# NomaDamas/AutoRAG-Research

Measured on AMD Instinct MI355X. Metric: queries/sec, higher is better.
Workload: dtype f32

## Files before the change

### autorag_research_amd/csrc/index.h

```cpp
#pragma once
#include <climits>
#include <hip/hip_runtime.h>

#include <algorithm>
#include <cmath>
#include <cstdio>
#include <cstring>
#include <mutex>
#include <string>
#include <vector>

#include "dev_common.h"
#include "mi355dr.h"

namespace mi355 {
template <class T, bool Pinned = false>
struct DevBuf {
    T* p = nullptr;
    size_t bytes = 0;
    DevBuf() = default;
    DevBuf(const DevBuf&) = delete;
    DevBuf& operator=(const DevBuf&) = delete;
    ~DevBuf() { release(); }
    void release() {
        if (p) (void)(Pinned ? hipHostFree(p) : hipFree(p));
        p = nullptr;
        bytes = 0;
    }
    hipError_t grow(size_t want) {
        if (want <= bytes) return hipSuccess;
        void* q = nullptr;
        const hipError_t e = Pinned ? hipHostMalloc(&q, want) : hipMalloc(&q, want);
        if (e != hipSuccess) return e;
        release();
        p = (T*)q;
        bytes = want;
        return hipSuccess;
    }
    void swap(DevBuf& o) {
        std::swap(p, o.p);
        std::swap(bytes, o.bytes);
    }
    operator T*() const { return p; }
};
template <class T>
using HostBuf = DevBuf<T, true>;

// ... 28 lines not shown
    int k = 0;
    int level = 0;
    bool screening = false;
    bool i8 = false;
    bool wide = false;
    int cap = 0;
    bool speculative = false;
    bool spec_eligible = false;
    int spec_m = 0;
    const char* refused = nullptr;
};
struct Pending {
    bool active = false;
    Event done;
    HostBuf<int> status_host;
    hipStream_t stream = nullptr;
    const float* q_dev = nullptr;
    int B = 0;
    Pass pass;
    double* out_dist = nullptr;
    int64_t* out_rows = nullptr;
};
struct RetryBufs {
    DevBuf<float> q;
    DevBuf<double> dist;
    DevBuf<int64_t> rows;
    DevBuf<int> map;
};
constexpr int kPendingRing = 4;

// ... 327 lines not shown
```

### autorag_research_amd/csrc/k_prep.h

```cpp
#pragma once
#include "dev_common.h"

namespace mi355 {

__global__ __launch_bounds__(64) void k_row_nrm2(const float* __restrict__ rows, int64_t row0, int64_t n, int d,
                                                  float* __restrict__ nrm2, unsigned* __restrict__ n2max,
                                                  const int64_t* __restrict__ ids) {
    __shared__ float tile[kStageFloats];
    const int lane = threadIdx.x;
    const int64_t j = (int64_t)blockIdx.x * kWave + lane;
    const bool live = j < n;
    const int64_t i = ids ? (live ? ids[j] : 0) : row0 + j;
    const float* my_row = live ? rows + i * (int64_t)d : nullptr;
    float acc = 0.0f;
    for (int k0 = 0; k0 < d; k0 += kStageCols) {
        stage_rows(tile, my_row, k0, d, lane);
        __syncthreads();
        const int kn = min(kStageCols, d - k0);
        const float* t = tile + lane * kStageLd;
        for (int k = 0; k < kn; ++k) acc = __builtin_fmaf(t[k], t[k], acc);
        __syncthreads();
    }
    if (live) nrm2[i] = acc;
    float m = (live && norm_is_regular(acc)) ? acc : 0.0f;
// ... 133 lines not shown
            if (!tight && i >= first_new) {
                const int slot = atomicAdd(irr8_count, 1);
                if (slot < kIrrCap) irr8_rows[slot] = (int32_t)i;
            }
        }
    }
    __syncthreads();
    if (threadIdx.x == 0) {
        float mx = 0.0f;
        for (int j = 0; j < kI8GroupRows; ++j) mx = fmaxf(mx, s_err[j]);
        grp[g].step = step;
        grp[g].err = mx;
    }
}

__global__ __launch_bounds__(64) void k_prep_queries(const float* __restrict__ q, int B, int d, int dpad, int metric,
                                                      QueryState st, int dpad8, int i8, float bf16_ec, int* status_or,
                                                      int* prune_skip, int cnt0, float cscale) {
    extern __shared__ float qs[];
    const int b = blockIdx.x;
    const int lane = threadIdx.x;
    if (b == 0 && lane == 0) {
        if (status_or) *status_or = 0;
        if (prune_skip) prune_skip[0] = prune_skip[1] = 0;
    }
    uint16_t* qh = st.qhat + (int64_t)b * dpad;
    if (b >= B) {
        for (int k = lane; k < dpad; k += kWave) qh[k] = 0;
        if (lane == 0) {
            st.qn[b] = 0.0f;
            st.thr[b] = __builtin_inff();
            st.cnt[b] = 0;
            st.carry[b] = 0;
            st.thr_used[b] = -__builtin_inff();
            st.best_n[b] = 0;
            st.thr_key[b] = 0;
            st.thr_row[b] = -1;
            st.status[b] = 0;
            st.E[b] = bf16_screen_bound(0.00390625f, bf16_ec, d, cscale);
            st.E16[b] = st.E[b];
            st.sc[b] = 0.0f;
            st.kq[b] = 1.0f;
        }
        if (i8)
            for (int k = lane; k < dpad8; k += kWave) st.qhat8[(int64_t)b * dpad8 + k] = 0;
        return;
    }
    const float* qr = q + (int64_t)b * d;
    for (int k = lane; k < d; k += kWave) qs[k] = qr[k];
    __syncthreads();
    float acc = 0.0f;
    for (int k = 0; k < d; ++k) acc = __builtin_fmaf(qs[k], qs[k], acc);
    const bool regular = norm_is_regular(acc);
    const float rq = regular ? 1.0f / sqrtf(acc) : 0.0f;
    float eq2 = 0.0f;
    for (int k = lane; k < dpad; k += kWave) {
        uint16_t v = 0;
        if (k < d && regular) {
            const float qh_f = qs[k] * rq;
            v = f32_to_bf16_rn(qh_f);
            const float e = qh_f - bf16_bits_to_f32(v);
            eq2 = __builtin_fmaf(e, e, eq2);
        }
        qh[k] = v;
// ... 50 lines not shown
```

### autorag_research_amd/csrc/k_select.h

```cpp
#pragma once
#include "dev_common.h"

namespace mi355 {

struct PruneArgs {
    const float* rows;
    const float* nrm2;
    const float* q;
    QueryState st;
    int32_t* cand_row;
    float* cand_val;
    const int* qlist;
    unsigned long long* stat;
    int cap, d, k, metric;
    int exact;
    const uint8_t* flag8;
    float cscale;
    const uint16_t* shadow16;
    int dpad;
    int round_a;
    int* skip_list;
    int skip_parity;
    int thr_only;
    int one_wave_only;
    int defer_b;
    SpecModel spec;
};

__device__ __forceinline__ float unit_sim(int metric, double dist, float inv_qn) {
    return metric == 0 ? (float)(1.0 - dist) : (float)(-dist) * inv_qn;
}
__device__ __forceinline__ float screen_threshold(int metric, double dist_k, float E, float nq) {
    if (metric == 0) return float_below((float)((1.0 - dist_k) - (double)E));
    const double u = -dist_k / sqrt((double)nq);
    return float_below((float)(u - fabs(u) * 4e-6 - (double)E));
}

constexpr int kPruneSmallThreads = 64, kPruneSmallSort = 1024;
constexpr int kPruneBigThreads = 256, kPruneBigSort = kSortMax;

__host__ __device__ inline size_t prune_qs_floats(int d) { return ((size_t)d + 3) / 4 * 4 + 16; }
// ... 37 lines not shown
        }
    }
#pragma unroll
    for (int j = 0; j < PER; ++j) {
        uint32_t kk = 0;
        if (j * T + tid < n_new) {
            if (v[j] != v[j]) kk = 0xFFFFFFFFu;
            else if (!f[j]) kk = f32_order_key(v[j]);
        }
        key[j] = kk;
        if (ROWS) rows_out[j] = r[j];
    }
}

template <int THREADS, int SORT>
__device__ __forceinline__ void prune_body(const PruneArgs& a, char* smem);

template <int THREADS, int SORT>
__global__ __launch_bounds__(THREADS) void k_prune(PruneArgs a) {
    extern __shared__ __attribute__((aligned(16))) char smem[];
    const bool list_mode = a.skip_list != nullptr && a.qlist == nullptr;
    const int tid = threadIdx.x;
    const int lane = tid & 63, wave = tid >> 6;
    int q = a.qlist ? a.qlist[blockIdx.x] : blockIdx.x;
    if (SORT == kPruneBigSort && list_mode) {
        if (blockIdx.x == 0 && tid == 0) a.skip_list[a.skip_parity ^ 1] = 0;
        const int n_left = a.skip_list[a.skip_parity];
        for (int i = blockIdx.x; i < n_left; i += gridDim.x) {
            PruneArgs b = a;
            b.skip_list = nullptr;
            b.qlist = a.skip_list + 2 + a.skip_parity * kQBlockMax + i - 0;
            b.qlist -= blockIdx.x;
            prune_body<THREADS, SORT>(b, smem);
            __syncthreads();
        }
        return;
    }
    prune_body<THREADS, SORT>(a, smem);
}

template <int THREADS, int SORT>
__device__ __forceinline__ void prune_body(const PruneArgs& a, char* smem) {
    constexpr int kWaves = THREADS / kWave;
    uint64_t* SK = (uint64_t*)smem;
    int32_t* SR = (int32_t*)(smem + (size_t)SORT * 8);
    char* X = smem + (size_t)SORT * 12;
    constexpr size_t xa = (size_t)kWaves * kStageFloats * sizeof(float), xb = (size_t)SORT * sizeof(float);
    constexpr size_t xbytes = xa > xb ? xa : xb;
    float* Lf = (float*)X;
    float* tiles = (float*)X;
    int32_t* R = (int32_t*)(X + xbytes);
    float* qs = (float*)(X + xbytes + (size_t)SORT * 4);
    int& s_cnt = *(int*)(X + xbytes + (size_t)SORT * 4 + (prune_qs_floats(a.d) - 16) * 4);
    float* q16 = qs + prune_qs_floats(a.d);
    const bool list_mode = a.skip_list != nullptr && a.qlist == nullptr;
    const int q = a.qlist ? a.qlist[blockIdx.x] : blockIdx.x;
    const int tid = threadIdx.x;
    const int lane = tid & 63, wave = tid >> 6;
    const int raw_cnt = a.st.cnt[q];
    const int n_best = a.st.best_n[q];
    if (raw_cnt == 0) return;
    if (a.exact && SORT < kPruneBigSort) return;
    auto leave_for_general = [&]() {
        if (a.one_wave_only) {
            if (tid == 0) {
                a.st.status[q] |= kStOverflow;
                a.st.cnt[q] = 0;
            }
            return;
        }
        if (list_mode && tid == 0) {
            const int i = atomicAdd(&a.skip_list[a.skip_parity], 1);
            a.skip_list[2 + a.skip_parity * kQBlockMax + i] = q;
        }
    };
    if (raw_cnt > a.cap) {
        if (SORT < kPruneBigSort) {
            leave_for_general();
            return;
        }
        if (tid == 0) {
            a.st.status[q] |= kStOverflow;
            a.st.cnt[q] = 0;
        }
        return;
    }
    if (n_best + raw_cnt > SORT) {
        if (SORT < kPruneBigSort) {
            leave_for_general();
            return;
        }
        if (tid == 0) {
            a.st.status[q] |= kStOverflow;
            a.st.cnt[q] = 0;
        }
        return;
    }
    const int n_new = raw_cnt;
    const int32_t* crow = a.cand_row + (int64_t)q * a.cap;
    const float* cval = a.cand_val + (int64_t)q * a.cap;
    uint64_t* bkey = a.st.best_key + (int64_t)q * kKMax;
    int32_t* brow = a.st.best_row + (int64_t)q * kKMax;
    const float nq = a.st.qn[q];
    const float inv_qn = 1.0f / sqrtf(nq);
    const float E = a.st.E[q];
    if (tid == 0) {
        a.stat[2 * q] += (unsigned long long)(n_new - a.st.carry[q]);
        a.st.carry[q] = 0;
    }

    int n_res;
// ... 204 lines not shown
                        a.st.thr_key[q] = wk;
                        a.st.thr_row[q] = R2[a.k - 1];
                    }
                    if (wk != kKeyNaN && !(a.st.status[q] & kStIrregular)) {
                        float thr = screen_threshold(a.metric, key_to_dist(wk), E, nq);
                        if (a.thr_only && a.spec.moments != nullptr) {
                            const double dist_t = a.metric == 0 ? 1.0 - (double)t_model : -(double)t_model * sqrt((double)nq);
                            const float thr_model = screen_threshold(a.metric, dist_t, E, nq);
                            if (thr_model > thr && thr_model < __builtin_inff()) thr = thr_model;
                            a.st.thr_used[q] = thr;
                        }
                        a.st.thr[q] = thr;
                    }
                }
            }
            return;
        }
    }
    if (!a.exact) {
        const int nLp = next_pow2(n_new);
        for (int i = tid; i < nLp; i += THREADS) {
            float v = -__builtin_inff();
            if (i < n_new) {
                v = cval[i];
                if (v != v) v = __builtin_inff();
                else if (a.flag8 && a.flag8[crow[i]]) v = -__builtin_inff();
            }
            Lf[i] = v;
            R[i] = i;
        }
        if (tid == 0) s_cnt = 0;
// ... 86 lines not shown
    for (int i = tid; i < n_keep; i += THREADS) {
        bkey[i] = SK[i];
        brow[i] = SR[i];
    }
    if (tid == 0) {
        a.st.best_n[q] = n_keep;
        a.st.cnt[q] = 0;
        if (n_keep >= a.k) {
            const uint64_t wk = SK[a.k - 1];
            a.st.thr_key[q] = wk;
            a.st.thr_row[q] = SR[a.k - 1];
            if (!a.exact && wk != kKeyNaN && !(a.st.status[q] & kStIrregular))
                a.st.thr[q] = screen_threshold(a.metric, key_to_dist(wk), E, nq);
        }
    }
}

__global__ __launch_bounds__(64) void k_emit_irregular(const int32_t* __restrict__ irr_rows, int irr_n, QueryState st,
                                                        int32_t* cand_row, float* cand_val, int cap, int skip_below) {
    const int q = blockIdx.x;
    if (st.status[q] & kStIrregular) return;
    for (int i = threadIdx.x; i < irr_n; i += blockDim.x) {
        if (irr_rows[i] < skip_below) continue;
        const int slot = atomicAdd(&st.cnt[q], 1);
        if (slot < cap) {
            cand_row[(int64_t)q * cap + slot] = irr_rows[i];
            cand_val[(int64_t)q * cap + slot] = __builtin_nanf("");
        }
    }
}

__global__ __launch_bounds__(64) void k_finalize(QueryState st, int k, int64_t row_offset, const int64_t* __restrict__ row_map,
                                                  double* out_dist, int64_t* out_rows, int* status_or, int spec_metric) {
    const int q = blockIdx.x;
    const int n = st.best_n[q];
    if (threadIdx.x == 0 && spec_metric >= 0 && !(st.status[q] & kStIrregular)) {
        float thr_final = -__builtin_inff();
        if (n >= k) {
            const uint64_t wk = st.best_key[(int64_t)q * kKMax + k - 1];
            if (wk != kKeyNaN) thr_final = screen_threshold(spec_metric, key_to_dist(wk), st.E[q], st.qn[q]);
        }
        if (n < k || thr_final < st.thr_used[q]) st.status[q] |= kStSpecMiss;
    }
    for (int s = threadIdx.x; s < k; s += blockDim.x) {
        if (s < n && st.best_row[(int64_t)q * kKMax + s] != kRowNone) {
            out_dist[(int64_t)q * k + s] = key_to_dist(st.best_key[(int64_t)q * kKMax + s]);
            const int32_t r = st.best_row[(int64_t)q * kKMax + s];
            out_rows[(int64_t)q * k + s] = row_map ? row_map[r] : (int64_t)r + row_offset;
        } else {
            out_dist[(int64_t)q * k + s] = __longlong_as_double(0x7FF8000000000000ll);
            out_rows[(int64_t)q * k + s] = -1;
        }
    }
    if (threadIdx.x == 0 && st.status[q] != 0) atomicOr(status_or, st.status[q]);
}

__global__ __launch_bounds__(256) void k_merge_topk(const double* __restrict__ dist_all,
                                                     const int64_t* __restrict__ rows_all, int64_t rank_stride, int world,
                                                     int B, int k, double* out_dist, int64_t* out_rows) {
    extern __shared__ __attribute__((aligned(16))) char smem[];
    uint64_t* SK = (uint64_t*)smem;
    const int np_ = next_pow2(world * k);
    int32_t* SI = (int32_t*)(smem + (size_t)np_ * 8);
    const int q = blockIdx.x;
    const int n = world * k;
    const int np = next_pow2(n);
    for (int i = threadIdx.x; i < np; i += blockDim.x) {
        if (i < n) {
            const int w = i / k, s = i % k;
            const int64_t src = (int64_t)w * rank_stride + (int64_t)q * k + s;
// ... 58 lines not shown
```

### autorag_research_amd/csrc/mi355dr.hip

```cpp
#include "index.h"
#include "k_prep.h"
#include "k_scan.h"
#include "k_scan_ids.h"
#include "subset_ids.h"
#include "screen_common.h"
#include "k_screen.h"
#include "k_screen256c.h"
#include "k_screen_rq.h"

#define MI355_RQ_FORMS(X) X(1) X(2) X(3) X(4) X(5) X(6)
inline bool screen_rq_has(int ksteps) { return ksteps >= 1 && ksteps <= 6; }
#include "k_screen_stream.h"
#include "k_select.h"
#include "k_prune_wide.h"
#include "k_update.h"
#include "k_compact.h"
#include "k_view.h"
#include "k_block.h"
#include "k_mmr.h"
#include "mmr_order.h"
#include "k_groups.h"
#include "k_fuse.h"
#include "k_range.h"
#include "k_rows.h"
// ... 225 lines not shown
    ps.screening = idx->n > 0 && screen_possible && path != MI355DR_PATH_SCAN;
    ps.wide = ps.screening && wide_ok(idx, k);
    ps.cap = !idx->cap_set && ps.wide ? kCandCapWide : idx->cap;
    if (idx->screen_dtype == MI355DR_SCREEN_I8 && !i8_available(idx) && path != MI355DR_PATH_SCAN)
        ps.refused = "int8 screen unavailable: too many rows outside the residual limit";
    else if (path == MI355DR_PATH_SCREEN && !screen_possible && idx->n > 0) ps.refused = no_screen;
    ps.spec_m = spec_m_of(k);
    ps.spec_eligible = level == 0 && ps.screening && !ps.wide && ps.spec_m > 0 && idx->speculate && idx->n >= idx->spec_min_rows &&
                       kSpecInflation * ps.spec_m * 4 <= 3 * (std::min(kPruneSmallSort, ps.cap) - k) &&
                       starter_sample_rows(idx, ps) > 0;
    ps.speculative = ps.spec_eligible && idx->spec_probation <= 0;
    return ps;
}
inline bool idle_i8(const mi355dr_index* idx) { return decide_pass(idx, idx->last_pass_k, 0, false).i8; }

int launch_prune(mi355dr_index* idx, hipStream_t s, const Pass& ps, int nblocks, const int* qlist, int exact,
                 bool thr_only = false, bool one_wave_only = false, bool defer_b = false, const SpecModel* spec = nullptr) {
    PruneArgs pa{};
    if (spec) pa.spec = *spec;
    pa.thr_only = thr_only ? 1 : 0;
    pa.one_wave_only = one_wave_only ? 1 : 0;
    pa.defer_b = defer_b && idx->defer_round_b ? 1 : 0;
    pa.rows = idx->rows;
    pa.nrm2 = idx->nrm2;
    pa.q = idx->qdev;
    pa.st = idx->st;
    pa.cand_row = idx->cand_row;
    pa.cand_val = idx->cand_val;
    pa.qlist = qlist;
    pa.stat = idx->stat_dev;
    pa.cap = ps.cap;
    pa.d = idx->dim;
    pa.k = ps.k;
    pa.metric = idx->metric;
    pa.exact = exact;
    pa.flag8 = (ps.i8 && (idx->irr8_n > 0 || idx->dead_n > 0)) ? idx->flag8 : nullptr;
    pa.cscale = idx->metric == MI355DR_METRIC_IP ? idx->cmax : 1.0f;
    pa.shadow16 = (ps.i8 && idx->metric == 0 && !exact && idx->prefilter16) ? idx->shadow : nullptr;
    pa.dpad = idx->dpad;
    pa.round_a = idx->round_a;
    if (!exact && ps.wide) {
        pa.shadow16 = nullptr;
        hipLaunchKernelGGL((k_prune_wide<2, 32>), dim3(nblocks), dim3(2 * kWave), prune_wide_lds_bytes(idx->dim, 2), s, pa);
        HIPCHECK(idx, hipGetLastError());
        return MI355DR_OK;
    }
    if (pa.cap > kCandCap) return fail(idx, MI355DR_E_INTERNAL, "general-form prune on a list stride above kCandCap");
    const bool list_mode = qlist == nullptr;
    pa.skip_list = list_mode ? idx->prune_skip : nullptr;
    pa.skip_parity = list_mode ? (idx->prune_parity ^= 1) : 0;
    hipLaunchKernelGGL((k_prune<kPruneSmallThreads, kPruneSmallSort>), dim3(nblocks), dim3(kPruneSmallThreads),
                       prune_lds_bytes(idx->dim, kPruneSmallThreads, kPruneSmallSort, pa.shadow16 ? idx->dpad : 0), s, pa);
    HIPCHECK(idx, hipGetLastError());
    if (one_wave_only) return MI355DR_OK;
    hipLaunchKernelGGL((k_prune<kPruneBigThreads, kPruneBigSort>), dim3(list_mode ? std::min(nblocks, 64) : nblocks),
                       dim3(kPruneBigThreads), prune_lds_bytes(idx->dim, kPruneBigThreads, kPruneBigSort, 0), s, pa);
    HIPCHECK(idx, hipGetLastError());
    return MI355DR_OK;
}

int launch_prep(mi355dr_index* idx, hipStream_t s, int B, int Bpad, int metric, bool i8, int cnt0 = 0) {
    hipLaunchKernelGGL(k_prep_queries, dim3(Bpad), dim3(64), (size_t)idx->dim * sizeof(float), s, idx->qdev, B, idx->dim,
                       idx->dpad, metric, idx->st, idx->dpad8, i8 ? 1 : 0, idx->bf16_ec, idx->status_or_dev,
                       idx->prune_skip, cnt0, idx->metric == MI355DR_METRIC_IP ? idx->cmax : 1.0f);
    idx->prune_parity = 0;
    HIPCHECK(idx, hipGetLastError());
    return MI355DR_OK;
}

inline int screen_tile(int B) { return B > kTileN ? kT2 : kTileM; }

constexpr int kRetryLevels = 2;

enum ScreenKernel { kKernTile = 0, kKernStream = 1, kKern256c = 2, kKernRq = 3 };
inline ScreenKernel screen_kernel_for(const mi355dr_index* idx, bool i8, int B, int64_t rows, bool emit_all) {
    const int tile = (emit_all || rows <= idx->small_chunk_rows) ? kTileM : screen_tile(B);
    const int row_bytes = i8 ? idx->dpad8 : idx->dpad * 2;
    const int ksteps = row_bytes / kRowB;
    if (tile == kT2) return i8 && idx->screen_rq && screen_rq_has(ksteps) ? kKernRq : kKern256c;
// ... 173 lines not shown
    const double zq = normal_quantile(1.0 - (double)ps.spec_m / (double)idx->n) + idx->spec_shift_milli / 1000.0;
    sm.zq = (float)zq;
    if (zq_out) *zq_out = zq;
    return sm;
}

PassPlan make_plan(const mi355dr_index* idx, const Pass& ps, int B) {
    const double budget = growth_budget(idx, ps.k, ps.i8);
    double growth = std::max(0.25, std::min((double)idx->chunk_growth, budget));
    if (B <= 64 && ps.level == 0 && idx->chunk_growth_set == 0) growth = std::max(growth, std::min(8.0, budget * kSmallBlockBudget));
    if (ps.level == 1) growth = std::max(0.25, growth * 0.5);
    if (ps.level >= 2) growth = 0.25;
    return plan_pass(idx, ps, B, growth);
}

int run_screen(mi355dr_index* idx, hipStream_t s, const Pass& ps, int B, const PassPlan& plan) {
    int64_t kept_all_below = 0;
    const bool i8 = ps.i8;
    const int side_n = i8 ? idx->irr8_n : idx->irr_n;
    constexpr int kSideMerge = 32;
    bool side_done = false;
    const bool lean = plan.sample > 0 && idx->prune_companion == 0;
    auto timed = [&](bool big, int64_t rows, auto&& launch) -> int {
        EventPair ev{};
        if (idx->profile) {
            ev = take_events(idx);
            HIPCHECK(idx, hipEventRecord(ev.a, s));
        }
        CHECK(launch());
        if (idx->profile) {
            HIPCHECK(idx, hipEventRecord(ev.b, s));
// ... 23 lines not shown
    }
    int64_t done = 0;
    for (size_t ci = 0; ci < plan.ends.size(); ++ci) {
        const int64_t end = plan.ends[ci];
        const bool emit_all = ci == 0 && plan.emit_all_first;
        if (emit_all) kept_all_below = end;
        const bool big = !emit_all && end - done > idx->small_chunk_rows && screen_tile(B) == kT2;
        const int64_t seen = ci == 0 ? (plan.sample > 0 ? plan.sample : end) : done;
        const double lanes = ps.speculative ? (double)kSpecInflation * ps.spec_m * 4096.0 / (double)idx->n
                                            : 8.0 * ps.k * 4096.0 / (double)std::max<int64_t>(seen, 1);
        int period = 1;
        while (period < 64 && period * 2 * lanes <= idx->screen_flush_lanes) period *= 2;
        const int flush_mask = idx->screen_flush_sync ? period - 1 : -1;
        CHECK(timed(big, end - done, [&] { return launch_screen(idx, s, i8, B, done, end, ps.cap, emit_all ? kEmitAll : 0, flush_mask); }));
        idx->s_chunks++;
        if (end >= idx->n && side_n > 0 && side_n <= kSideMerge) {
            hipLaunchKernelGGL(k_emit_irregular, dim3(B), dim3(64), 0, s, i8 ? idx->irr8_rows : idx->irr_rows, side_n, idx->st,
                               idx->cand_row, idx->cand_val, ps.cap, (int)kept_all_below);
            HIPCHECK(idx, hipGetLastError());
            side_done = true;
        }
        const bool last = end >= idx->n && (side_n == 0 || side_done);
        CHECK(launch_prune(idx, s, ps, B, nullptr, 0, false, lean, !last));
        done = end;
    }
    if (side_n > 0 && !side_done) {
        hipLaunchKernelGGL(k_emit_irregular, dim3(B), dim3(64), 0, s, i8 ? idx->irr8_rows : idx->irr_rows, side_n, idx->st,
                           idx->cand_row, idx->cand_val, ps.cap, (int)kept_all_below);
        HIPCHECK(idx, hipGetLastError());
        CHECK(launch_prune(idx, s, ps, B, nullptr, 0, false, lean));
    }
    idx->s_passes++;
    return MI355DR_OK;
}

int launch_scan(mi355dr_index* idx, hipStream_t s, const int* qlist, int nq, int cap, int64_t r0, int64_t r1,
                const int32_t* ids = nullptr) {
    ScanArgs sa{};
    sa.rows = idx->rows;
    sa.nrm2 = idx->nrm2;
    sa.q = idx->qdev;
    sa.st = idx->st;
    sa.cand_row = idx->cand_row;
    sa.cand_val = idx->cand_val;
    sa.qlist = qlist;
// ... 57 lines not shown
                }
            }
            done = end;
            chunk = std::max<int64_t>(chunk, done * (idx->chunk_growth_set ? idx->chunk_growth : 63));
        }
    }
    if (ids) HIPCHECK(idx, hipStreamSynchronize(s));
    else idx->s_fallback_queries += nq_all;
    return MI355DR_OK;
}

int subset_block(mi355dr_index* idx, hipStream_t s, const float* q_dev, int B, int k, int64_t m, double* out_dist_dev,
                 int64_t* out_rows_dev) {
    const Pass ps = decide_pass(idx, k, 0, true);
    idx->last_pass_k = k;
    if (q_dev != idx->qdev)
        HIPCHECK(idx, hipMemcpyAsync(idx->qdev, q_dev, (size_t)B * idx->dim * sizeof(float), hipMemcpyDeviceToDevice, s));
    CHECK(launch_prep(idx, s, B, (int)round_up(B, screen_tile(B)), idx->metric, ps.i8));
    std::vector<int> all(B);
    for (int i = 0; i < B; ++i) all[i] = i;
    if (m > 0) CHECK(run_scan(idx, s, ps, all, m, idx->subset_ids));
    hipLaunchKernelGGL(k_finalize, dim3(B), dim3(64), 0, s, idx->st, k, idx->row_offset, idx->view_row_map.p, out_dist_dev,
                       out_rows_dev, idx->status_or_dev, -1);
    HIPCHECK(idx, hipGetLastError());
    HIPCHECK(idx, hipMemcpyAsync(idx->status_host, idx->st.status, (size_t)kQBlockMax * sizeof(int), hipMemcpyDeviceToHost, s));
    HIPCHECK(idx, hipStreamSynchronize(s));
    for (int i = 0; i < B; ++i)
        if (idx->status_host[i] & kStOverflow)
            return fail(idx, MI355DR_E_INTERNAL, "subset scan: query " + std::to_string(i) + " lost a candidate chunk");
    return MI355DR_OK;
}

int pending_alloc(mi355dr_index* idx, Pending& p) {
    HIPCHECK(idx, p.status_host.grow((kQBlockMax + 1) * sizeof(int)));
    HIPCHECK(idx, p.done.create(hipEventDisableTiming));
    return MI355DR_OK;
}

int enqueue_block(mi355dr_index* idx, hipStream_t s, const float* q_dev, int B, int k, double* out_dist_dev,
                  int64_t* out_rows_dev, Pending& p, int level = 0, bool force_scan = false) {
    CHECK(ensure_qstate(idx));
    CHECK(pending_alloc(idx, p));
    idx->last_pass_k = k;
    if (level == 0 && idx->screen_dtype == MI355DR_SCREEN_AUTO && k >= idx->i8_demoted_k && --idx->i8_probation <= 0)
        idx->i8_demoted_k = INT_MAX;
    const int Bpad = (int)round_up(B, screen_tile(B));
    const Pass ps = decide_pass(idx, k, level, force_scan, "screen path unavailable (metric or too many irregular rows)");
    if (ps.refused) return fail(idx, MI355DR_E_UNSUPPORTED, ps.refused);
    if (idx->spec_probation > 0 && ps.spec_eligible) idx->spec_probation--;
    if (q_dev != idx->qdev)
        HIPCHECK(idx, hipMemcpyAsync(idx->qdev, q_dev, (size_t)B * idx->dim * sizeof(float), hipMemcpyDeviceToDevice, s));
    PassPlan plan;
    if (ps.screening) plan = make_plan(idx, ps, B);
    CHECK(launch_prep(idx, s, B, Bpad, idx->metric, ps.i8, starter_count(plan)));
    if (idx->n > 0) {
        if (ps.screening) {
            CHECK(run_screen(idx, s, ps, B, plan));
        } else {
            std::vector<int> all(B);
            for (int i = 0; i < B; ++i) all[i] = i;
            CHECK(run_scan(idx, s, ps, all, idx->n));
        }
    }
    hipLaunchKernelGGL(k_finalize, dim3(B), dim3(64), 0, s, idx->st, k, idx->row_offset, idx->view_row_map.p, out_dist_dev,
                       out_rows_dev, idx->status_or_dev, ps.speculative && idx->n > 0 ? idx->metric : -1);
    HIPCHECK(idx, hipGetLastError());
    HIPCHECK(idx, hipMemcpyAsync(p.status_host, idx->st.status, (size_t)(kQBlockMax + 1) * sizeof(int), hipMemcpyDeviceToHost, s));
    HIPCHECK(idx, hipEventRecord(p.done, s));
    p.active = true;
    p.stream = s;
    p.q_dev = q_dev;
    p.B = B;
    p.pass = ps;
    p.out_dist = out_dist_dev;
    p.out_rows = out_rows_dev;
    return MI355DR_OK;
}

int search_block(mi355dr_index* idx, hipStream_t s, const float* q_dev, int B, int k, double* out_dist_dev,
                 int64_t* out_rows_dev, int level = 0, bool force_scan = false);

int complete_block(mi355dr_index* idx, Pending& p) {
    if (!p.active) return MI355DR_OK;
    p.active = false;
    HIPCHECK(idx, hipEventSynchronize(p.done));
    drain_events(idx);
    if (!p.pass.screening) {
        for (int i = 0; i < p.B; ++i)
            if (p.status_host[i] & kStOverflow)
                return fail(idx, MI355DR_E_INTERNAL, "exact scan: query " + std::to_string(i) + " lost a candidate chunk");
        return MI355DR_OK;
    }
    if (p.status_host[kQBlockMax] == 0) return MI355DR_OK;
    hipStream_t s = p.stream;
    const int B = p.B, k = p.pass.k, level = p.pass.level;
    std::vector<int> sub;
    int n_todo = 0;
    {
        std::vector<int> retry;
        for (int i = 0; i < B; ++i) {
            const int st = p.status_host[i];
            if (st == 0) continue;
            if (p.pass.speculative && !(st & kStIrregular)) {
                if (st & kStOverflow) idx->s_spec_overflow_queries++;
                else if (st & kStSpecMiss) idx->s_spec_miss_queries++;
            }
            if (level < kRetryLevels && !(st & kStIrregular)) retry.push_back(i);
            else sub.push_back(i);
// ... 1245 lines not shown

int range_block(mi355dr_index* idx, hipStream_t s, const float* q_dev, int nb, const double* radius, int m, double* od,
                int64_t* orow, int64_t* ocount) {
    const Pass ps = decide_pass(idx, 1, 0, false, "screen path unavailable (too many irregular rows)");
    if (ps.refused) return fail(idx, MI355DR_E_UNSUPPORTED, ps.refused);
    const int cap = ps.cap;
    const bool i8 = ps.i8, use_screen = ps.screening;
    const int64_t chunk = round_up(std::max<int64_t>(idx->range_chunk_rows, kT2), kT2);
    std::vector<RangeSpan> spans;
    for (int64_t r0 = 0; r0 < idx->n; r0 += chunk) spans.push_back(RangeSpan{r0, std::min(idx->n, r0 + chunk)});
    const int n_main = (int)spans.size();
    const int R = range_slots_for(idx, m);
    const int64_t pairs = (int64_t)nb * std::max(n_main, 1);
    CHECK(ensure_range(idx, nb, R, m, pairs));
    const RangeState rs = range_state(idx, R, pairs);
    if (q_dev != idx->qdev)
        HIPCHECK(idx, hipMemcpyAsync(idx->qdev, q_dev, (size_t)nb * idx->dim * sizeof(float), hipMemcpyDeviceToDevice, s));
    CHECK(launch_prep(idx, s, nb, (int)round_up(nb, screen_tile(nb)), idx->metric, i8));
    HIPCHECK(idx, hipMemcpyAsync(idx->rng.radius.p, radius, (size_t)nb * sizeof(double), hipMemcpyHostToDevice, s));
    HIPCHECK(idx, hipMemsetAsync(idx->rng.redo.p, 0, 2 * sizeof(int), s));
    HIPCHECK(idx, hipMemsetAsync(idx->rng.stat.p, 0, 2 * sizeof(unsigned long long), s));
    hipLaunchKernelGGL(k_range_prep, dim3((nb + kRangeThreads - 1) / kRangeThreads), dim3(kRangeThreads), 0, s,
                       (const double*)idx->rng.radius.p, nb, idx->metric, use_screen ? 1 : 0, idx->st, rs);
    HIPCHECK(idx, hipGetLastError());
    std::vector<int> all(nb);
    for (int i = 0; i < nb; ++i) all[i] = i;
    if (use_screen) {
        for (int i = 0; i < n_main; ++i) {
            CHECK(launch_screen(idx, s, i8, nb, spans[i].r0, spans[i].r1, cap, 0, idx->screen_flush_sync ? 15 : -1));
            CHECK(launch_range_collect(idx, s, ps, rs, kRangeFormScreen, nb, nullptr, i, spans[i].r0));
        }
        const int side_n = i8 ? idx->irr8_n : idx->irr_n;
        const int32_t* side = i8 ? idx->irr8_rows.p : idx->irr_rows.p;
// ... 141 lines not shown
    for (int b0 = 0; b0 < B; b0 += kQBlockMax) {
        const int nb = std::min(kQBlockMax, B - b0);
        const BlockOut<int64_t> o = block_outputs(idx, io, b0);
        HIPCHECK(idx, hipMemcpyAsync(idx->rowq.ids.p, row_ids + b0, (size_t)nb * sizeof(int64_t), hipMemcpyHostToDevice, s));
        hipLaunchKernelGGL(k_rows_gather, dim3(nb), dim3(kRowsThreads), 0, s, (const int64_t*)idx->rowq.ids.p, idx->row_offset,
                           idx->n, (const float*)idx->rows.p, (const float*)idx->nrm2.p, idx->dim, idx->rowq.q.p,
                           idx->rowq.valid.p, idx->rowq.pair_q.p, idx->rowq.pair_row.p, idx->rowq.skipped_dev.p);
        HIPCHECK(idx, hipGetLastError());
        if (idx->n > 0 && !range) {
            CHECK(search_block(idx, s, idx->rowq.q.p, nb, stride, idx->rowq.cand_dist.p, idx->rowq.cand_rows.p));
        } else if (idx->n > 0) {
            rad.assign(radius + b0, radius + b0 + nb);
            for (int b = 0; b < nb; ++b)
                if (subset_local_row(row_ids[b0 + b], idx->row_offset, idx->n) < 0) rad[b] = -INFINITY;
            HIPCHECK(idx, hipMemcpyAsync(idx->rowq.radius.p, rad.data(), (size_t)nb * sizeof(double), hipMemcpyHostToDevice, s));
            HIPCHECK(idx, hipMemcpyAsync(idx->qdev, idx->rowq.q.p, (size_t)nb * idx->dim * sizeof(float), hipMemcpyDeviceToDevice, s));
            CHECK(launch_prep(idx, s, nb, (int)round_up(nb, screen_tile(nb)), idx->metric, idle_i8(idx)));
            CHECK(launch_rescore(idx, s, idx->rowq.pair_q.p, idx->rowq.pair_row.p, nb, idx->rowq.self_dot.p, idx->rowq.self_dist.p));
            CHECK(range_block(idx, s, idx->rowq.q.p, nb, rad.data(), stride, idx->rowq.cand_dist.p, idx->rowq.cand_rows.p,
                              idx->rowq.cand_count.p));
        }
        hipLaunchKernelGGL(k_rows_drop, dim3(nb), dim3(kRowsThreads), 0, s, (const double*)idx->rowq.cand_dist.p,
                           (const int64_t*)idx->rowq.cand_rows.p, stride, (const int64_t*)idx->rowq.ids.p,
                           (const int*)idx->rowq.valid.p, kout, include_self ? 1 : 0,
                           range ? (const int64_t*)idx->rowq.cand_count.p : nullptr, (const double*)idx->rowq.self_dist.p,
                           (const double*)idx->rowq.radius.p, o.dist, o.rows, o.count);
        HIPCHECK(idx, hipGetLastError());
        CHECK(block_return(idx, io, b0, nb, o));
        HIPCHECK(idx, hipStreamSynchronize(s));
    }
    unsigned long long skipped = 0;
    HIPCHECK(idx, hipMemcpy(&skipped, idx->rowq.skipped_dev.p, sizeof(skipped), hipMemcpyDeviceToHost));
// ... 160 lines not shown
    for (int b0 = 0; b0 < B; b0 += kQBlockMax) {
        const int nb = std::min(kQBlockMax, B - b0);
        const int64_t qw = shard_rows_qwords(nb, d), vw = shard_rows_vwords(nb), words = shard_rows_words(nb, d);
        const size_t lists = (size_t)2 * nb * stride + (range ? nb : 0);
        CHECK(shard_reserve_words(idx, std::max((size_t)words, lists)));
        float* pay_q = (float*)idx->shd.send.p;
        int* pay_valid = (int*)(idx->shd.send.p + qw);
        double* pay_self = (double*)(idx->shd.send.p + qw + vw);
        HIPCHECK(idx, hipMemsetAsync(idx->shd.send.p, 0, (size_t)words * sizeof(int64_t), s));
        HIPCHECK(idx, hipMemcpyAsync(idx->rowq.ids.p, row_ids + b0, (size_t)nb * sizeof(int64_t), hipMemcpyHostToDevice, s));
        hipLaunchKernelGGL(k_rows_gather, dim3(nb), dim3(kRowsThreads), 0, s, (const int64_t*)idx->rowq.ids.p, idx->row_offset,
                           idx->n, (const float*)idx->rows.p, (const float*)idx->nrm2.p, d, pay_q, pay_valid, idx->rowq.pair_q.p,
                           idx->rowq.pair_row.p, idx->shd.local_skipped.p);
        HIPCHECK(idx, hipGetLastError());
        if (range && idx->n > 0) {
            HIPCHECK(idx, hipMemcpyAsync(idx->qdev, pay_q, (size_t)nb * d * sizeof(float), hipMemcpyDeviceToDevice, s));
            CHECK(launch_prep(idx, s, nb, (int)round_up(nb, screen_tile(nb)), idx->metric, idle_i8(idx)));
            CHECK(launch_rescore(idx, s, idx->rowq.pair_q.p, idx->rowq.pair_row.p, nb, idx->rowq.self_dot.p, pay_self));
        }
        CHECK(shard_gather(idx, s, idx->shd.send.p, idx->shd.recv.p, (size_t)words * sizeof(int64_t)));
        hipLaunchKernelGGL(k_shard_rows_fold, dim3(nb), dim3(kShardThreads), 0, s, (const int64_t*)idx->shd.recv.p, words, world, nb,
                           d, idx->rowq.q.p, idx->rowq.valid.p, idx->rowq.self_dist.p, idx->rowq.skipped_dev.p);
        HIPCHECK(idx, hipGetLastError());
        if (!range) {
            CHECK(shard_topk_block(idx, s, idx->rowq.q.p, nb, stride, idx->rowq.cand_dist.p, idx->rowq.cand_rows.p));
        } else {
            valid.resize(nb);
            HIPCHECK(idx, hipMemcpyAsync(valid.data(), idx->rowq.valid.p, (size_t)nb * sizeof(int), hipMemcpyDeviceToHost, s));
            HIPCHECK(idx, hipStreamSynchronize(s));
            rad.assign(radius + b0, radius + b0 + nb);
            for (int b = 0; b < nb; ++b)
                if (!valid[b]) rad[b] = -INFINITY;
// ... 675 lines not shown
```

Before: 164,200.

## Fuse finalize and side-row emission into prune, fold query copy into prep

Drops the separate device-to-device query copy by having the prep kernel write the copy while it loads. On the screening path it appends irregular side rows inside the prune kernel instead of a separate k_emit_irregular launch. The last prune then finalizes each query in-kernel and writes per-query status straight into mapped pinned host memory, which removes the k_finalize launch and the status memcpy. The cost is more prune-kernel complexity, host-side OR over per-query status, and reliance on mapped host writes being visible after the event.

```diff
diff --git a/autorag_research_amd/csrc/index.h b/autorag_research_amd/csrc/index.h
--- a/autorag_research_amd/csrc/index.h
+++ b/autorag_research_amd/csrc/index.h
@@ -30,7 +30,7 @@
     hipError_t grow(size_t want) {
         if (want <= bytes) return hipSuccess;
         void* q = nullptr;
-        const hipError_t e = Pinned ? hipHostMalloc(&q, want) : hipMalloc(&q, want);
+        const hipError_t e = Pinned ? hipHostMalloc(&q, want, hipHostMallocMapped) : hipMalloc(&q, want);
         if (e != hipSuccess) return e;
         release();
         p = (T*)q;
@@ -89,6 +89,7 @@
     bool active = false;
     Event done;
     HostBuf<int> status_host;
+    bool status_fused = false;
     hipStream_t stream = nullptr;
     const float* q_dev = nullptr;
     int B = 0;
diff --git a/autorag_research_amd/csrc/k_prep.h b/autorag_research_amd/csrc/k_prep.h
--- a/autorag_research_amd/csrc/k_prep.h
+++ b/autorag_research_amd/csrc/k_prep.h
@@ -171,9 +171,9 @@
     }
 }
 
-__global__ __launch_bounds__(64) void k_prep_queries(const float* __restrict__ q, int B, int d, int dpad, int metric,
-                                                      QueryState st, int dpad8, int i8, float bf16_ec, int* status_or,
-                                                      int* prune_skip, int cnt0, float cscale) {
+__global__ __launch_bounds__(64) void k_prep_queries(const float* __restrict__ q, float* __restrict__ q_copy, int B, int d,
+                                                      int dpad, int metric, QueryState st, int dpad8, int i8, float bf16_ec,
+                                                      int* status_or, int* prune_skip, int cnt0, float cscale) {
     extern __shared__ float qs[];
     const int b = blockIdx.x;
     const int lane = threadIdx.x;
@@ -204,7 +204,11 @@
         return;
     }
     const float* qr = q + (int64_t)b * d;
-    for (int k = lane; k < d; k += kWave) qs[k] = qr[k];
+    for (int k = lane; k < d; k += kWave) {
+        const float v = qr[k];
+        qs[k] = v;
+        if (q_copy != nullptr) q_copy[(int64_t)b * d + k] = v;
+    }
     __syncthreads();
     float acc = 0.0f;
     for (int k = 0; k < d; ++k) acc = __builtin_fmaf(qs[k], qs[k], acc);
diff --git a/autorag_research_amd/csrc/k_select.h b/autorag_research_amd/csrc/k_select.h
--- a/autorag_research_amd/csrc/k_select.h
+++ b/autorag_research_amd/csrc/k_select.h
@@ -2,6 +2,17 @@
 #include "dev_common.h"
 
 namespace mi355 {
+
+struct FinalizeArgs {
+    int k;
+    int spec_metric;
+    int64_t row_offset;
+    const int64_t* row_map;
+    double* out_dist;
+    int64_t* out_rows;
+    int* status_or;
+    int* status_host;
+};
 
 struct PruneArgs {
     const float* rows;
@@ -25,6 +36,10 @@
     int one_wave_only;
     int defer_b;
     SpecModel spec;
+    FinalizeArgs fin;
+    const int32_t* side_rows;
+    int side_n;
+    int side_skip_below;
 };
 
 __device__ __forceinline__ float unit_sim(int metric, double dist, float inv_qn) {
@@ -92,7 +107,9 @@
 }
 
 template <int THREADS, int SORT>
-__device__ __forceinline__ void prune_body(const PruneArgs& a, char* smem);
+__device__ __forceinline__ bool prune_body(const PruneArgs& a, char* smem);
+
+__device__ __forceinline__ void finalize_query(const QueryState& st, const FinalizeArgs& f, int q, int tid, int nthreads);
 
 template <int THREADS, int SORT>
 __global__ __launch_bounds__(THREADS) void k_prune(PruneArgs a) {
@@ -109,16 +126,22 @@
             b.skip_list = nullptr;
             b.qlist = a.skip_list + 2 + a.skip_parity * kQBlockMax + i - 0;
             b.qlist -= blockIdx.x;
+            b.side_n = 0;
             prune_body<THREADS, SORT>(b, smem);
             __syncthreads();
+            if (a.fin.k > 0) finalize_query(a.st, a.fin, a.skip_list[2 + a.skip_parity * kQBlockMax + i], tid, THREADS);
         }
         return;
     }
-    prune_body<THREADS, SORT>(a, smem);
+    const bool settled = prune_body<THREADS, SORT>(a, smem);
+    if (a.fin.k > 0 && settled) {
+        __syncthreads();
+        finalize_query(a.st, a.fin, q, tid, THREADS);
+    }
 }
 
 template <int THREADS, int SORT>
-__device__ __forceinline__ void prune_body(const PruneArgs& a, char* smem) {
+__device__ __forceinline__ bool prune_body(const PruneArgs& a, char* smem) {
     constexpr int kWaves = THREADS / kWave;
     uint64_t* SK = (uint64_t*)smem;
     int32_t* SR = (int32_t*)(smem + (size_t)SORT * 8);
@@ -135,44 +158,56 @@
     const int q = a.qlist ? a.qlist[blockIdx.x] : blockIdx.x;
     const int tid = threadIdx.x;
     const int lane = tid & 63, wave = tid >> 6;
-    const int raw_cnt = a.st.cnt[q];
+    int raw_cnt = a.st.cnt[q];
     const int n_best = a.st.best_n[q];
-    if (raw_cnt == 0) return;
-    if (a.exact && SORT < kPruneBigSort) return;
-    auto leave_for_general = [&]() {
+    if (a.side_n > 0 && !(a.st.status[q] & kStIrregular)) {
+        const int32_t row = lane < a.side_n ? a.side_rows[lane] : 0;
+        const bool want = lane < a.side_n && row >= a.side_skip_below;
+        const unsigned long long bal = __builtin_amdgcn_ballot_w64(want);
+        const int slot = raw_cnt + (int)__builtin_amdgcn_mbcnt_hi((unsigned)(bal >> 32), __builtin_amdgcn_mbcnt_lo((unsigned)bal, 0));
+        if (wave == 0 && want && slot < a.cap) {
+            a.cand_row[(int64_t)q * a.cap + slot] = row;
+            a.cand_val[(int64_t)q * a.cap + slot] = __builtin_nanf("");
+        }
+        raw_cnt += __builtin_popcountll(bal);
+        if (tid == 0) a.st.cnt[q] = raw_cnt;
+        __syncthreads();
+    }
+    if (raw_cnt == 0) return true;
+    if (a.exact && SORT < kPruneBigSort) return false;
+    auto leave_for_general = [&]() -> bool {
         if (a.one_wave_only) {
             if (tid == 0) {
                 a.st.status[q] |= kStOverflow;
                 a.st.cnt[q] = 0;
             }
-            return;
+            return true;
         }
         if (list_mode && tid == 0) {
             const int i = atomicAdd(&a.skip_list[a.skip_parity], 1);
             a.skip_list[2 + a.skip_parity * kQBlockMax + i] = q;
         }
+        return false;
     };
     if (raw_cnt > a.cap) {
         if (SORT < kPruneBigSort) {
-            leave_for_general();
-            return;
+            return leave_for_general();
         }
         if (tid == 0) {
             a.st.status[q] |= kStOverflow;
             a.st.cnt[q] = 0;
         }
-        return;
+        return true;
     }
     if (n_best + raw_cnt > SORT) {
         if (SORT < kPruneBigSort) {
-            leave_for_general();
-            return;
+            return leave_for_general();
         }
         if (tid == 0) {
             a.st.status[q] |= kStOverflow;
             a.st.cnt[q] = 0;
         }
-        return;
+        return true;
     }
     const int n_new = raw_cnt;
     const int32_t* crow = a.cand_row + (int64_t)q * a.cap;
@@ -407,7 +442,7 @@
                     }
                 }
             }
-            return;
+            return true;
         }
     }
     if (!a.exact) {
@@ -524,6 +559,7 @@
                 a.st.thr[q] = screen_threshold(a.metric, key_to_dist(wk), E, nq);
         }
     }
+    return true;
 }
 
 __global__ __launch_bounds__(64) void k_emit_irregular(const int32_t* __restrict__ irr_rows, int irr_n, QueryState st,
@@ -540,30 +576,37 @@
     }
 }
 
-__global__ __launch_bounds__(64) void k_finalize(QueryState st, int k, int64_t row_offset, const int64_t* __restrict__ row_map,
-                                                  double* out_dist, int64_t* out_rows, int* status_or, int spec_metric) {
-    const int q = blockIdx.x;
+__device__ __forceinline__ void finalize_query(const QueryState& st, const FinalizeArgs& f, int q, int tid, int nthreads) {
+    const int k = f.k;
     const int n = st.best_n[q];
-    if (threadIdx.x == 0 && spec_metric >= 0 && !(st.status[q] & kStIrregular)) {
+    for (int s = tid; s < k; s += nthreads) {
+        if (s < n && st.best_row[(int64_t)q * kKMax + s] != kRowNone) {
+            f.out_dist[(int64_t)q * k + s] = key_to_dist(st.best_key[(int64_t)q * kKMax + s]);
+            const int32_t r = st.best_row[(int64_t)q * kKMax + s];
+            f.out_rows[(int64_t)q * k + s] = f.row_map ? f.row_map[r] : (int64_t)r + f.row_offset;
+        } else {
+            f.out_dist[(int64_t)q * k + s] = __longlong_as_double(0x7FF8000000000000ll);
+            f.out_rows[(int64_t)q * k + s] = -1;
+        }
+    }
+    if (tid != 0) return;
+    int status = st.status[q];
+    if (f.spec_metric >= 0 && !(status & kStIrregular)) {
         float thr_final = -__builtin_inff();
         if (n >= k) {
             const uint64_t wk = st.best_key[(int64_t)q * kKMax + k - 1];
-            if (wk != kKeyNaN) thr_final = screen_threshold(spec_metric, key_to_dist(wk), st.E[q], st.qn[q]);
-        }
-        if (n < k || thr_final < st.thr_used[q]) st.status[q] |= kStSpecMiss;
-    }
-    for (int s = threadIdx.x; s < k; s += blockDim.x) {
-        if (s < n && st.best_row[(int64_t)q * kKMax + s] != kRowNone) {
-            out_dist[(int64_t)q * k + s] = key_to_dist(st.best_key[(int64_t)q * kKMax + s]);
-            const int32_t r = st.best_row[(int64_t)q * kKMax + s];
-            out_rows[(int64_t)q * k + s] = row_map ? row_map[r] : (int64_t)r + row_offset;
-        } else {
-            out_dist[(int64_t)q * k + s] = __longlong_as_double(0x7FF8000000000000ll);
-            out_rows[(int64_t)q * k + s] = -1;
-        }
-    }
-    if (threadIdx.x == 0 && st.status[q] != 0) atomicOr(status_or, st.status[q]);
-}
+            if (wk != kKeyNaN) thr_final = screen_threshold(f.spec_metric, key_to_dist(wk), st.E[q], st.qn[q]);
+        }
+        if (n < k || thr_final < st.thr_used[q]) {
+            status |= kStSpecMiss;
+            st.status[q] = status;
+        }
+    }
+    if (f.status_host != nullptr) f.status_host[q] = status;
+    else if (status != 0) atomicOr(f.status_or, status);
+}
+
+__global__ __launch_bounds__(64) void k_finalize(QueryState st, FinalizeArgs f) { finalize_query(st, f, blockIdx.x, threadIdx.x, blockDim.x); }
 
 __global__ __launch_bounds__(256) void k_merge_topk(const double* __restrict__ dist_all,
                                                      const int64_t* __restrict__ rows_all, int64_t rank_stride, int world,
diff --git a/autorag_research_amd/csrc/mi355dr.hip b/autorag_research_amd/csrc/mi355dr.hip
--- a/autorag_research_amd/csrc/mi355dr.hip
+++ b/autorag_research_amd/csrc/mi355dr.hip
@@ -263,10 +263,27 @@
 }
 inline bool idle_i8(const mi355dr_index* idx) { return decide_pass(idx, idx->last_pass_k, 0, false).i8; }
 
+inline FinalizeArgs finalize_args(const mi355dr_index* idx, int k, int spec_metric, double* out_dist_dev, int64_t* out_rows_dev) {
+    FinalizeArgs f{};
+    f.k = k;
+    f.spec_metric = spec_metric;
+    f.row_offset = idx->row_offset;
+    f.row_map = idx->view_row_map.p;
+    f.out_dist = out_dist_dev;
+    f.out_rows = out_rows_dev;
+    f.status_or = idx->status_or_dev;
+    return f;
+}
+
 int launch_prune(mi355dr_index* idx, hipStream_t s, const Pass& ps, int nblocks, const int* qlist, int exact,
-                 bool thr_only = false, bool one_wave_only = false, bool defer_b = false, const SpecModel* spec = nullptr) {
+                 bool thr_only = false, bool one_wave_only = false, bool defer_b = false, const SpecModel* spec = nullptr,
+                 const FinalizeArgs* fin = nullptr, const int32_t* side_rows = nullptr, int side_n = 0, int side_skip_below = 0) {
     PruneArgs pa{};
+    pa.side_rows = side_rows;
+    pa.side_n = side_n;
+    pa.side_skip_below = side_skip_below;
     if (spec) pa.spec = *spec;
+    if (fin) pa.fin = *fin;
     pa.thr_only = thr_only ? 1 : 0;
     pa.one_wave_only = one_wave_only ? 1 : 0;
     pa.defer_b = defer_b && idx->defer_round_b ? 1 : 0;
@@ -289,6 +306,7 @@
     pa.dpad = idx->dpad;
     pa.round_a = idx->round_a;
     if (!exact && ps.wide) {
+        if (fin || side_n > 0) return fail(idx, MI355DR_E_INTERNAL, "the two-wave prune neither finalizes nor appends side rows");
         pa.shadow16 = nullptr;
         hipLaunchKernelGGL((k_prune_wide<2, 32>), dim3(nblocks), dim3(2 * kWave), prune_wide_lds_bytes(idx->dim, 2), s, pa);
         HIPCHECK(idx, hipGetLastError());
@@ -296,6 +314,7 @@
     }
     if (pa.cap > kCandCap) return fail(idx, MI355DR_E_INTERNAL, "general-form prune on a list stride above kCandCap");
     const bool list_mode = qlist == nullptr;
+    if ((fin || side_n > 0) && !list_mode) return fail(idx, MI355DR_E_INTERNAL, "a finalizing prune walks the whole block");
     pa.skip_list = list_mode ? idx->prune_skip : nullptr;
     pa.skip_parity = list_mode ? (idx->prune_parity ^= 1) : 0;
     hipLaunchKernelGGL((k_prune<kPruneSmallThreads, kPruneSmallSort>), dim3(nblocks), dim3(kPruneSmallThreads),
@@ -308,10 +327,12 @@
     return MI355DR_OK;
 }
 
-int launch_prep(mi355dr_index* idx, hipStream_t s, int B, int Bpad, int metric, bool i8, int cnt0 = 0) {
-    hipLaunchKernelGGL(k_prep_queries, dim3(Bpad), dim3(64), (size_t)idx->dim * sizeof(float), s, idx->qdev, B, idx->dim,
-                       idx->dpad, metric, idx->st, idx->dpad8, i8 ? 1 : 0, idx->bf16_ec, idx->status_or_dev,
-                       idx->prune_skip, cnt0, idx->metric == MI355DR_METRIC_IP ? idx->cmax : 1.0f);
+int launch_prep(mi355dr_index* idx, hipStream_t s, int B, int Bpad, int metric, bool i8, int cnt0 = 0, const float* q_dev = nullptr) {
+    const bool own = q_dev == nullptr || q_dev == idx->qdev.p;
+    hipLaunchKernelGGL(k_prep_queries, dim3(Bpad), dim3(64), (size_t)idx->dim * sizeof(float), s, own ? idx->qdev.p : q_dev,
+                       own ? (float*)nullptr : idx->qdev.p, B, idx->dim, idx->dpad, metric, idx->st, idx->dpad8, i8 ? 1 : 0,
+                       idx->bf16_ec, idx->status_or_dev, idx->prune_skip.p, cnt0,
+                       idx->metric == MI355DR_METRIC_IP ? idx->cmax : 1.0f);
     idx->prune_parity = 0;
     HIPCHECK(idx, hipGetLastError());
     return MI355DR_OK;
@@ -515,7 +536,7 @@
     return plan_pass(idx, ps, B, growth);
 }
 
-int run_screen(mi355dr_index* idx, hipStream_t s, const Pass& ps, int B, const PassPlan& plan) {
+int run_screen(mi355dr_index* idx, hipStream_t s, const Pass& ps, int B, const PassPlan& plan, const FinalizeArgs* fin = nullptr) {
     int64_t kept_all_below = 0;
     const bool i8 = ps.i8;
     const int side_n = i8 ? idx->irr8_n : idx->irr_n;
@@ -569,21 +590,27 @@
         const int flush_mask = idx->screen_flush_sync ? period - 1 : -1;
         CHECK(timed(big, end - done, [&] { return launch_screen(idx, s, i8, B, done, end, ps.cap, emit_all ? kEmitAll : 0, flush_mask); }));
         idx->s_chunks++;
+        bool side_in_prune = false;
         if (end >= idx->n && side_n > 0 && side_n <= kSideMerge) {
-            hipLaunchKernelGGL(k_emit_irregular, dim3(B), dim3(64), 0, s, i8 ? idx->irr8_rows : idx->irr_rows, side_n, idx->st,
-                               idx->cand_row, idx->cand_val, ps.cap, (int)kept_all_below);
-            HIPCHECK(idx, hipGetLastError());
+            side_in_prune = !ps.wide;
+            if (!side_in_prune) {
+                hipLaunchKernelGGL(k_emit_irregular, dim3(B), dim3(64), 0, s, i8 ? idx->irr8_rows : idx->irr_rows, side_n, idx->st,
+                                   idx->cand_row, idx->cand_val, ps.cap, (int)kept_all_below);
+                HIPCHECK(idx, hipGetLastError());
+            }
             side_done = true;
         }
         const bool last = end >= idx->n && (side_n == 0 || side_done);
-        CHECK(launch_prune(idx, s, ps, B, nullptr, 0, false, lean, !last));
+        CHECK(launch_prune(idx, s, ps, B, nullptr, 0, false, lean, !last, nullptr, last ? fin : nullptr,
+                           side_in_prune ? (i8 ? idx->irr8_rows.p : idx->irr_rows.p) : nullptr, side_in_prune ? side_n : 0,
+                           (int)kept_all_below));
         done = end;
     }
     if (side_n > 0 && !side_done) {
         hipLaunchKernelGGL(k_emit_irregular, dim3(B), dim3(64), 0, s, i8 ? idx->irr8_rows : idx->irr_rows, side_n, idx->st,
                            idx->cand_row, idx->cand_val, ps.cap, (int)kept_all_below);
         HIPCHECK(idx, hipGetLastError());
-        CHECK(launch_prune(idx, s, ps, B, nullptr, 0, false, lean));
+        CHECK(launch_prune(idx, s, ps, B, nullptr, 0, false, lean, false, nullptr, fin));
     }
     idx->s_passes++;
     return MI355DR_OK;
@@ -671,14 +698,11 @@
                  int64_t* out_rows_dev) {
     const Pass ps = decide_pass(idx, k, 0, true);
     idx->last_pass_k = k;
-    if (q_dev != idx->qdev)
-        HIPCHECK(idx, hipMemcpyAsync(idx->qdev, q_dev, (size_t)B * idx->dim * sizeof(float), hipMemcpyDeviceToDevice, s));
-    CHECK(launch_prep(idx, s, B, (int)round_up(B, screen_tile(B)), idx->metric, ps.i8));
+    CHECK(launch_prep(idx, s, B, (int)round_up(B, screen_tile(B)), idx->metric, ps.i8, 0, q_dev));
     std::vector<int> all(B);
     for (int i = 0; i < B; ++i) all[i] = i;
     if (m > 0) CHECK(run_scan(idx, s, ps, all, m, idx->subset_ids));
-    hipLaunchKernelGGL(k_finalize, dim3(B), dim3(64), 0, s, idx->st, k, idx->row_offset, idx->view_row_map.p, out_dist_dev,
-                       out_rows_dev, idx->status_or_dev, -1);
+    hipLaunchKernelGGL(k_finalize, dim3(B), dim3(64), 0, s, idx->st, finalize_args(idx, k, -1, out_dist_dev, out_rows_dev));
     HIPCHECK(idx, hipGetLastError());
     HIPCHECK(idx, hipMemcpyAsync(idx->status_host, idx->st.status, (size_t)kQBlockMax * sizeof(int), hipMemcpyDeviceToHost, s));
     HIPCHECK(idx, hipStreamSynchronize(s));
@@ -705,26 +729,29 @@
     const Pass ps = decide_pass(idx, k, level, force_scan, "screen path unavailable (metric or too many irregular rows)");
     if (ps.refused) return fail(idx, MI355DR_E_UNSUPPORTED, ps.refused);
     if (idx->spec_probation > 0 && ps.spec_eligible) idx->spec_probation--;
-    if (q_dev != idx->qdev)
-        HIPCHECK(idx, hipMemcpyAsync(idx->qdev, q_dev, (size_t)B * idx->dim * sizeof(float), hipMemcpyDeviceToDevice, s));
     PassPlan plan;
     if (ps.screening) plan = make_plan(idx, ps, B);
-    CHECK(launch_prep(idx, s, B, Bpad, idx->metric, ps.i8, starter_count(plan)));
+    CHECK(launch_prep(idx, s, B, Bpad, idx->metric, ps.i8, starter_count(plan), q_dev));
+    FinalizeArgs fin = finalize_args(idx, k, ps.speculative && idx->n > 0 ? idx->metric : -1, out_dist_dev, out_rows_dev);
+    const bool fused = idx->n > 0 && ps.screening && !ps.wide;
     if (idx->n > 0) {
         if (ps.screening) {
-            CHECK(run_screen(idx, s, ps, B, plan));
+            if (fused) fin.status_host = p.status_host;
+            CHECK(run_screen(idx, s, ps, B, plan, fused ? &fin : nullptr));
         } else {
             std::vector<int> all(B);
             for (int i = 0; i < B; ++i) all[i] = i;
             CHECK(run_scan(idx, s, ps, all, idx->n));
         }
     }
-    hipLaunchKernelGGL(k_finalize, dim3(B), dim3(64), 0, s, idx->st, k, idx->row_offset, idx->view_row_map.p, out_dist_dev,
-                       out_rows_dev, idx->status_or_dev, ps.speculative && idx->n > 0 ? idx->metric : -1);
-    HIPCHECK(idx, hipGetLastError());
-    HIPCHECK(idx, hipMemcpyAsync(p.status_host, idx->st.status, (size_t)(kQBlockMax + 1) * sizeof(int), hipMemcpyDeviceToHost, s));
+    if (!fused) {
+        hipLaunchKernelGGL(k_finalize, dim3(B), dim3(64), 0, s, idx->st, fin);
+        HIPCHECK(idx, hipGetLastError());
+        HIPCHECK(idx, hipMemcpyAsync(p.status_host, idx->st.status, (size_t)(kQBlockMax + 1) * sizeof(int), hipMemcpyDeviceToHost, s));
+    }
     HIPCHECK(idx, hipEventRecord(p.done, s));
     p.active = true;
+    p.status_fused = fused;
     p.stream = s;
     p.q_dev = q_dev;
     p.B = B;
@@ -748,7 +775,12 @@
                 return fail(idx, MI355DR_E_INTERNAL, "exact scan: query " + std::to_string(i) + " lost a candidate chunk");
         return MI355DR_OK;
     }
-    if (p.status_host[kQBlockMax] == 0) return MI355DR_OK;
+    int status_or = p.status_host[kQBlockMax];
+    if (p.status_fused) {
+        status_or = 0;
+        for (int i = 0; i < p.B; ++i) status_or |= p.status_host[i];
+    }
+    if (status_or == 0) return MI355DR_OK;
     hipStream_t s = p.stream;
     const int B = p.B, k = p.pass.k, level = p.pass.level;
     std::vector<int> sub;
@@ -2024,9 +2056,7 @@
     const int64_t pairs = (int64_t)nb * std::max(n_main, 1);
     CHECK(ensure_range(idx, nb, R, m, pairs));
     const RangeState rs = range_state(idx, R, pairs);
-    if (q_dev != idx->qdev)
-        HIPCHECK(idx, hipMemcpyAsync(idx->qdev, q_dev, (size_t)nb * idx->dim * sizeof(float), hipMemcpyDeviceToDevice, s));
-    CHECK(launch_prep(idx, s, nb, (int)round_up(nb, screen_tile(nb)), idx->metric, i8));
+    CHECK(launch_prep(idx, s, nb, (int)round_up(nb, screen_tile(nb)), idx->metric, i8, 0, q_dev));
     HIPCHECK(idx, hipMemcpyAsync(idx->rng.radius.p, radius, (size_t)nb * sizeof(double), hipMemcpyHostToDevice, s));
     HIPCHECK(idx, hipMemsetAsync(idx->rng.redo.p, 0, 2 * sizeof(int), s));
     HIPCHECK(idx, hipMemsetAsync(idx->rng.stat.p, 0, 2 * sizeof(unsigned long long), s));
@@ -2198,8 +2228,7 @@
             for (int b = 0; b < nb; ++b)
                 if (subset_local_row(row_ids[b0 + b], idx->row_offset, idx->n) < 0) rad[b] = -INFINITY;
             HIPCHECK(idx, hipMemcpyAsync(idx->rowq.radius.p, rad.data(), (size_t)nb * sizeof(double), hipMemcpyHostToDevice, s));
-            HIPCHECK(idx, hipMemcpyAsync(idx->qdev, idx->rowq.q.p, (size_t)nb * idx->dim * sizeof(float), hipMemcpyDeviceToDevice, s));
-            CHECK(launch_prep(idx, s, nb, (int)round_up(nb, screen_tile(nb)), idx->metric, idle_i8(idx)));
+            CHECK(launch_prep(idx, s, nb, (int)round_up(nb, screen_tile(nb)), idx->metric, idle_i8(idx), 0, idx->rowq.q.p));
             CHECK(launch_rescore(idx, s, idx->rowq.pair_q.p, idx->rowq.pair_row.p, nb, idx->rowq.self_dot.p, idx->rowq.self_dist.p));
             CHECK(range_block(idx, s, idx->rowq.q.p, nb, rad.data(), stride, idx->rowq.cand_dist.p, idx->rowq.cand_rows.p,
                               idx->rowq.cand_count.p));
@@ -2390,8 +2419,7 @@
                            idx->rowq.pair_row.p, idx->shd.local_skipped.p);
         HIPCHECK(idx, hipGetLastError());
         if (range && idx->n > 0) {
-            HIPCHECK(idx, hipMemcpyAsync(idx->qdev, pay_q, (size_t)nb * d * sizeof(float), hipMemcpyDeviceToDevice, s));
-            CHECK(launch_prep(idx, s, nb, (int)round_up(nb, screen_tile(nb)), idx->metric, idle_i8(idx)));
+            CHECK(launch_prep(idx, s, nb, (int)round_up(nb, screen_tile(nb)), idx->metric, idle_i8(idx), 0, pay_q));
             CHECK(launch_rescore(idx, s, idx->rowq.pair_q.p, idx->rowq.pair_row.p, nb, idx->rowq.self_dot.p, pay_self));
         }
         CHECK(shard_gather(idx, s, idx->shd.send.p, idx->shd.recv.p, (size_t)words * sizeof(int64_t)));
```

New measurement: 164,300 (median of 2 runs). About the same (+0.1%).
